# MKMaS-GUET/MTVAF

Measured on AMD Instinct MI355X. Metric: training sentences/sec (fwd+bwd), higher is better.
Workload: dtype fp32 (3xbf16 split products, fp32 accumulate)

## Files before the change

include/mtvaf_hip.h:

```cpp
#ifndef MTVAF_HIP_H
#define MTVAF_HIP_H

#include <stddef.h>
#include <stdint.h>

#ifdef __cplusplus
extern "C" {
#endif

typedef void* mtvaf_stream_t;

#define MTVAF_OK 0
#define MTVAF_ERR_SHAPE (-1)
#define MTVAF_ERR_ALIGN (-2)
#define MTVAF_ERR_ARG (-3)
#define MTVAF_ERR_WORKSPACE (-4)

#define MTVAF_KC 0
#define MTVAF_KM 1
#define MTVAF_EPI_NONE 0
#define MTVAF_EPI_GELU 1
#define MTVAF_EPI_TANH 2
#define MTVAF_EPI_DGELU 3
#define MTVAF_EPI_DTANH 4
// ... 265 lines not shown
typedef struct {
  float* dh;
  float* dh1;
  void *df, *dpre, *da, *dctx, *dqkv;
  float *part, *partq, *partkv;
  float* delta;
  float *dwqkv, *dbqkv, *dwo, *dbo, *dg1, *db1, *dw1, *dbi1, *dw2, *dbi2, *dg2, *db2;
  float *dpk, *dpv;
  void* ws_main; size_t ws_main_bytes;
  void* ws_side; size_t ws_side_bytes;
  const int* klist;
  const int* kcnt;
  int zero_tail;
  float *lnpart2, *lnpart1;
  void *df_p, *dpre_p, *da_p, *dqkv_p;
} mtvaf_layer_grads_t;

int mtvaf_encoder_layer_fwd(const mtvaf_layer_t* layer, mtvaf_stream_t stream);
int mtvaf_encoder_layer_bwd(const mtvaf_layer_t* layer, const mtvaf_layer_grads_t* grads, mtvaf_stream_t main,
                            mtvaf_stream_t side, int settle);
size_t mtvaf_layer_struct_bytes(int which );

int mtvaf_adamw(float* p, const float* g, float* m, float* v, long n, float lr, double beta1, double beta2, float eps,
                float weight_decay, float bc1, float bc2_sqrt, float grad_scale, void* p_bf16, int max_blocks,
                mtvaf_stream_t stream);
int mtvaf_adamw_planes(float* p, const float* g, float* m, float* v, long n, float lr, double beta1, double beta2, float eps,
                       float weight_decay, float bc1, float bc2_sqrt, float grad_scale, int nseg, const long* seg_begin,
                       const int* seg_rows, const int* seg_cols, void* const* seg_img, int max_blocks, mtvaf_stream_t stream);
int mtvaf_adamw_multi(int count, float* const* p, const float* const* g, float* const* m, float* const* v,
                      const long* n, float lr, double beta1, double beta2, float eps, float weight_decay, float bc1,
// ... 11 lines not shown
```

mtvaf_amd/csrc/executor.hip:

```cpp
#include "common.h"

#include <cstdlib>

#include <cstddef>

extern "C" {
int mtvaf_gemm_f32(int layout_a, int layout_b, const float* A, int lda, const float* B, int ldb, float* C, int ldc, int M,
                   int N, int K, const float* bias, int epi, float* aux, int ldaux, int accumulate, int allow_split,
                   void* workspace, size_t workspace_bytes, int cfg, int splits, hipStream_t stream);
int mtvaf_gemm_bf16x(int layout_a, int layout_b, const void* A, int lda, const void* B, int ldb, float* C32, int ldc32,
                     void* C16, int ldc16, int M, int N, int K, const float* bias, int epi, void* aux16, int ldaux,
                     int accumulate, float* colpart, int allow_split, void* workspace, size_t workspace_bytes, int tile,
                     int splits, int stages, hipStream_t stream);
int mtvaf_gemm_f32_dw_group(int n, const float* const* A, const int* lda, const float* const* B, const int* ldb, float* const* C,
                            const int* ldc, const int* M, const int* N, int K, const int* klist, const int* kcnt,
                            void* workspace, size_t workspace_bytes, int splits, hipStream_t stream);
int mtvaf_gemm_f32_dw_group_bias(int n, const float* const* A, const int* lda, const float* const* B, const int* ldb, float* const* C,
                                 const int* ldc, const int* M, const int* N, int K, const int* klist, const int* kcnt,
                                 float* const* dbias, void* workspace, size_t workspace_bytes, int splits, hipStream_t stream);
int mtvaf_streamk_attached(hipStream_t stream);
int mtvaf_gemm_bf16x_dw_group(int n, const void* const* A, const int* lda, const void* const* B, const int* ldb, float* const* C32,
                              const int* ldc32, const int* M, const int* N, int K, hipStream_t stream);
int mtvaf_gemm_bf16x_ktiles(int layout_a, int layout_b, const void* A, int lda, const void* B, int ldb, float* C32, int ldc32,
                            void* C16, int ldc16, int M, int N, int K, const float* bias, int epi, void* aux16, int ldaux,
// ... 190 lines not shown
struct mtvaf_layer_grads_t {
  float* dh;
  float* dh1;
  void *df, *dpre, *da, *dctx, *dqkv;
  float *part, *partq, *partkv;
  float* delta;
  float *dwqkv, *dbqkv, *dwo, *dbo, *dg1, *db1, *dw1, *dbi1, *dw2, *dbi2, *dg2, *db2;
  float *dpk, *dpv;
  void* ws_main; size_t ws_main_bytes;
  void* ws_side; size_t ws_side_bytes;
  const int* klist;
  const int* kcnt;
  int zero_tail;
  float *lnpart2, *lnpart1;
  void *df_p, *dpre_p, *da_p, *dqkv_p;
};

static int p16_ep(int lb, const void* Ap, const void* Wp, void* Cp, float* colpart, int M, int N, int K, const float* bias, int epi, float* aux,
                  int ldaux, hipStream_t st) {
  const long ap = (long)M * 64, akt = (long)3 * M * 64;
  const long bp = (long)(lb == 0 ? N : K) * 64, bkt = lb == 0 ? (long)3 * N * 64 : 2048, bc = lb == 0 ? 0 : (long)12 * K * 64;
  return mtvaf_gemm_f32p_ep(0, Ap, ap, 64, akt, 0, lb, Wp, bp, 64, bkt, bc, nullptr, 0, Cp, colpart, M, N, K, bias, epi, aux, ldaux, 0, st);
}

static bool planes_mode(const mtvaf_layer_t* L) {
  return !L->bf16 && L->cu && L->x_p && L->cx_p && L->h1_p && L->act_p && L->wqkv_h && L->wo_h && L->w1_h && L->w2_h && L->Mp % 128 == 0 &&
         L->H % 128 == 0 && L->I % 128 == 0 && L->ws;
}

static int dense_ln_fwd_p(const void* Ap, int K, const void* Wp, const float* bias, float* x_out, const float* res, const float* gamma,
                          const float* beta, float* out, float* mean, float* rstd, int M, int H, float eps, float p_drop, uint64_t seed,
// ... 120 lines not shown
                               nullptr, 0, nullptr, 0, 0, -1, 0, mainS));
    MTVAF_TRY(ln_bwd_forked(g->dh1, L->a, L->x, L->g1, L->mean1, L->rstd1, nullptr, g->dh, g->dg1, g->db1, g->dbo, M, H, L->p_hidden,
                            L->seed, L->offset + 1, g->lnpart1, g->ws_main, g->ws_main_bytes, g->da, mainS, side));
    if (!grp) MTVAF_TRY(mtvaf_gemm_bf16x_ktiles(X_KM, X_KM, g->da, H, L->cx, H, g->dwo, H, nullptr, 0, H, H, M, nullptr, X_EPI_NONE, nullptr, 0, 0,
                               nullptr, 1, g->ws_side, g->ws_side_bytes, 0, -1, 0, g->klist, g->kcnt, side));
    MTVAF_TRY(mtvaf_gemm_bf16x(X_KC, X_KM, g->da, H, L->wo_h, H, nullptr, 0, g->dctx, H, M, H, H, nullptr, X_EPI_NONE, nullptr, 0, 0,
                               nullptr, 0, nullptr, 0, 0, -1, 0, mainS));
    if (L->cu) {
      MTVAF_TRY(mtvaf_prefix_attn_bf16_varlen_bwd(g->dctx, L->qkv, L->pk, L->pv, L->cu, L->Mp - L->Mv, L->cx, L->lse, g->dqkv, g->dpk,
                                                  g->dpv, g->partq, g->partkv, B, S, P, NH, 64, L->p_attn, L->seed, L->offset, mainS));
    } else {
      MTVAF_TRY(mtvaf_prefix_attn_bf16_bwd_tail(g->dctx, L->qkv, L->pk, L->pv, L->addmask, L->cx, L->lse, g->dqkv, g->dpk, g->dpv, g->partq,
                                                g->partkv, B, S, P, NH, 64, L->p_attn, L->seed, L->offset,
                                                (g->klist != nullptr || g->zero_tail) ? 1 : 0, mainS));
    }
    MTVAF_TRY(fork_to(mainS, side));
    MTVAF_TRY(mtvaf_colsum_small(g->partq, B * ((S + 63) / 64), H, g->dbqkv, 0, side));
    MTVAF_TRY(mtvaf_colsum_small(g->partkv, B * ((P + S + 63) / 64), 2 * H, g->dbqkv + H, 0, side));
    if (!grp) MTVAF_TRY(mtvaf_gemm_bf16x_ktiles(X_KM, X_KM, g->dqkv, 3 * H, L->x_h, H, g->dwqkv, H, nullptr, 0, 3 * H, H, M, nullptr, X_EPI_NONE,
                               nullptr, 0, 0, nullptr, 1, g->ws_side, g->ws_side_bytes, 0, -1, 0, g->klist, g->kcnt, side));
    if (grp) {
      const void* const As[4] = {g->df, g->dpre, g->da, g->dqkv};
      const void* const Bs[4] = {L->act, L->h1_h, L->cx, L->x_h};
      float* const Cs[4] = {static_cast<float*>(g->dw2), static_cast<float*>(g->dw1), static_cast<float*>(g->dwo), static_cast<float*>(g->dwqkv)};
      const int lda[4] = {H, I, H, 3 * H}, ldb[4] = {I, H, H, H}, ldc[4] = {I, H, H, H};
      const int Ms[4] = {H, I, H, 3 * H}, Ns[4] = {I, H, H, H};
      MTVAF_TRY(mtvaf_gemm_bf16x_dw_group(4, As, lda, Bs, ldb, Cs, ldc, Ms, Ns, M, side));
    }
    MTVAF_TRY(mtvaf_gemm_bf16x(X_KC, X_KM, g->dqkv, 3 * H, L->wqkv_h, H, g->dh, H, nullptr, 0, M, H, 3 * H, nullptr, X_EPI_NONE,
                               nullptr, 0, 1, nullptr, 0, nullptr, 0, 0, -1, 0, mainS));
// ... 9 lines not shown
    const float* act = static_cast<const float*>(L->act);
    if (planes_mode(L)) {
      if (!g->df_p || !g->dpre_p || !g->da_p || !g->dqkv_p || !g->part || !g->lnpart2 || !g->lnpart1 || !g->ws_main) return MTVAF_ERR_ARG;
      MTVAF_TRY(mtvaf_dropout_res_ln_bwd_rows_planes(g->dh, nullptr, 0, L->f, L->h1, L->g2, L->mean2, L->rstd2, nullptr, g->dh1, 0, M, H,
                                                     L->p_hidden, L->seed, L->offset + 2, g->lnpart2, g->df_p, mainS));
      MTVAF_TRY(p16_ep(1, g->df_p, L->w2_h, g->dpre_p, g->part, M, I, H, nullptr, X_EPI_DGELU, pre, I, mainS));
      int ns1 = 1;
      MTVAF_TRY(p16(1, g->dpre_p, L->w1_h, g->dh1, H, M, H, I, nullptr, X_EPI_NONE, nullptr, 0, 1, g->ws_main, g->ws_main_bytes, &ns1, mainS));
      MTVAF_TRY(mtvaf_dropout_res_ln_bwd_rows_planes(g->dh1, static_cast<const float*>(g->ws_main), ns1 > 1 ? ns1 : 0, L->a, L->x, L->g1,
                                                     L->mean1, L->rstd1, nullptr, g->dh, 0, M, H, L->p_hidden, L->seed, L->offset + 1,
                                                     g->lnpart1, g->da_p, mainS));
      MTVAF_TRY(p16(1, g->da_p, L->wo_h, dctx, H, M, H, H, nullptr, X_EPI_NONE, nullptr, 0, 0, g->ws_main, g->ws_main_bytes, nullptr, mainS));
      MTVAF_TRY(mtvaf_prefix_attn_varlen_bwd_planes(dctx, qkv, static_cast<const float*>(L->pk), static_cast<const float*>(L->pv), L->cu,
                                                    L->Mp - L->Mv, cx, L->lse, g->delta, dqkv, g->dpk, g->dpv, B, S, P, NH, 64, L->p_attn,
                                                    L->seed, L->offset, g->dqkv_p, M, mainS));
      MTVAF_TRY(fork_to(mainS, side));
      {
        const void* const As[4] = {g->df_p, g->dpre_p, g->da_p, g->dqkv_p};
        const void* const Bs[4] = {L->act_p, L->h1_p, L->cx_p, L->x_p};
        float* const Cs[4] = {g->dw2, g->dw1, g->dwo, g->dwqkv};
        const int ldc[4] = {I, H, H, H}, Ms[4] = {H, I, H, 3 * H}, Ns[4] = {I, H, H, H};
        long strides[32];
        for (int i = 0; i < 8; ++i) {
          strides[4 * i] = (long)M * 64; strides[4 * i + 1] = 64; strides[4 * i + 2] = 2048; strides[4 * i + 3] = (long)12 * M * 64;
        }
        const float* js[8]; float* jd[8]; int jr[8], jc[8], jl[8], nj = 0;
        auto job = [&](const float* src, int rows, int cols, int ld, float* dst) {
          if (dst) { js[nj] = src; jr[nj] = rows; jc[nj] = cols; jl[nj] = ld; jd[nj] = dst; ++nj; }
        };
        job(dqkv, M, 3 * H, 3 * H, g->dbqkv);
// ... 37 lines not shown
                              L->offset + 1, g->lnpart1, g->ws_main, g->ws_main_bytes, nullptr, mainS, side));
    }
    if (!grp) MTVAF_TRY(mtvaf_gemm_f32_ktiles(X_KM, X_KM, da, H, cx, H, g->dwo, H, H, H, M, nullptr, X_EPI_NONE, nullptr, 0, 0, 1, g->ws_side,
                             g->ws_side_bytes, -1, -1, g->klist, g->kcnt, side));
    MTVAF_TRY(mtvaf_gemm_f32(X_KC, X_KM, da, H, L->wo, H, dctx, H, M, H, H, nullptr, X_EPI_NONE, nullptr, 0, 0, 1, g->ws_main,
                             g->ws_main_bytes, -1, -1, mainS));
    if (L->cu) {
      MTVAF_TRY(mtvaf_prefix_attn_varlen_bwd(dctx, qkv, static_cast<const float*>(L->pk), static_cast<const float*>(L->pv), L->cu,
                                             L->Mp - L->Mv, cx, L->lse, g->delta, dqkv, g->dpk, g->dpv, B, S, P, NH, 64, L->p_attn,
                                             L->seed, L->offset, mainS));
    } else {
      MTVAF_TRY(mtvaf_prefix_attn_bwd_tail(dctx, qkv, static_cast<const float*>(L->pk), static_cast<const float*>(L->pv), L->addmask, cx,
                                           L->lse, g->delta, dqkv, g->dpk, g->dpv, B, S, P, NH, 64, L->p_attn, L->seed, L->offset,
                                           (g->klist != nullptr || g->zero_tail) ? 1 : 0, mainS));
    }
    MTVAF_TRY(fork_to(mainS, side));
    if (!grp) MTVAF_TRY(mtvaf_colsum(dqkv, M, 3 * H, 3 * H, g->dbqkv, 0, g->ws_side, g->ws_side_bytes, side));
    if (!grp) MTVAF_TRY(mtvaf_gemm_f32_ktiles(X_KM, X_KM, dqkv, 3 * H, L->x, H, g->dwqkv, H, 3 * H, H, M, nullptr, X_EPI_NONE, nullptr, 0, 0, 1,
                             g->ws_side, g->ws_side_bytes, -1, -1, g->klist, g->kcnt, side));
    if (grp) {
      const float* const As[4] = {df, dpre, da, dqkv};
      const float* const Bs[4] = {act, static_cast<const float*>(L->h1), cx, static_cast<const float*>(L->x)};
      float* const Cs[4] = {g->dw2, g->dw1, g->dwo, g->dwqkv};
      const int lda[4] = {H, I, H, 3 * H}, ldb[4] = {I, H, H, H}, ldc[4] = {I, H, H, H};
      const int Ms[4] = {H, I, H, 3 * H}, Ns[4] = {I, H, H, H};
      float* const dbs[4] = {nullptr, g->dbi1, nullptr, g->dbqkv};
      MTVAF_TRY(mtvaf_gemm_f32_dw_group_bias(4, As, lda, Bs, ldb, Cs, ldc, Ms, Ns, M, g->klist, g->kcnt, dbs, g->ws_side, g->ws_side_bytes, -1,
                                             side));
    }
    MTVAF_TRY(mtvaf_gemm_f32(X_KC, X_KM, dqkv, 3 * H, L->wqkv, H, g->dh, H, M, H, 3 * H, nullptr, X_EPI_NONE, nullptr, 0, 1, 1,
// ... 10 lines not shown
```

mtvaf_amd/engine.py:

```python
from __future__ import annotations

import ctypes
import os
from typing import List, Optional

import torch

from . import hip



class _Rng:

    def __init__(self):
        self.offset = 0
        self.stream = 0

    def set_stream(self, stream: int):
        self.stream = int(stream)

    def seed(self) -> int:
        return (int(torch.initial_seed()) ^ (self.stream * 0x9E3779B97F4A7C15)) & 0xFFFFFFFFFFFFFFFF

    def next(self, n: int = 1) -> int:
# ... 174 lines not shown

N_LAYER_PARAMS = 16


DW_SIDE_STREAM = os.environ.get("MTVAF_DW_STREAM", "1") != "0"
DW_STREAM_MIN_ROWS = 1024
_side_streams = {}


def _side_stream(device) -> "torch.cuda.Stream":
    key = torch.device(device).index or 0
    st = _side_streams.get(key)
    if st is None:
        st = _side_streams[key] = torch.cuda.Stream(device=device)
    return st


NATIVE_EXEC = os.environ.get("MTVAF_NATIVE_EXEC", "1") != "0"
DIRECT_GRADS = os.environ.get("MTVAF_DIRECT_GRADS", "1") != "0"
UNPAD = os.environ.get("MTVAF_UNPAD", "1") != "0"


class padding_free:

    def __init__(self, on: bool):
        self.on = bool(on)

    def __enter__(self):
        global UNPAD
        self.was, UNPAD = UNPAD, self.on
# ... 315 lines not shown
    gviews = grad_sink.acquire(params) if grad_sink is not None else None
    if grad_sink is not None:
        grad_sink.token_rows = M
    direct = gviews is not None and DIRECT_GRADS and not _has_grad_hooks(params)
    if direct and _ddp_without_gradsync(grad_sink):
        direct = False
        if not _warned_ddp[0]:
            _warned_ddp[0] = True
            import warnings
            warnings.warn("mtvaf_amd: torch.distributed is initialised with several ranks but no mtvaf_amd.parallel.GradSync is attached "
                          "to this encoder; encoder gradients are returned through autograd (as with MTVAF_DIRECT_GRADS=0) so that a "
                          "DistributedDataParallel reducer sees them.  Use GradSync for the overlapped per-layer exchange.")
    pgrads: List[Optional[torch.Tensor]] = [None] * len(params)
    main = torch.cuda.current_stream()
    side = _side_stream(dev) if (DW_SIDE_STREAM and need_param_grads and M >= DW_STREAM_MIN_ROWS) else None
    main_h = hip._st()
    if side is not None:
        with torch.cuda.stream(side):
            side_h = hip._st()
            ws_side = hip.workspace(_exec_workspace_bytes(M, H, I, use_h), dev)
    else:
        side_h, ws_side = main_h, None
    ws_main = hip.workspace(_exec_workspace_bytes(M, H, I, use_h), dev)
    if ws_side is None:
        ws_side = ws_main
    if use_h and need_param_grads:
        _streamk_on(side, dev)
    (flay, _), (blay, btotal) = _fwd_layout(M, H, I, B, NH, S, use_h, planes), _bwd_layout(M, H, I, B, NH, S, Pn, use_h, planes)
    o_h2, o_h2h, o_h2p = dict(flay)["h2"], dict(flay)["h2_h"], dict(flay)["h2_p"]
    fn = hip.lib().mtvaf_encoder_layer_bwd
# ... 65 lines not shown
            gs = w._gst = hip.LayerGradsStruct()
        barena = torch.empty(btotal, dtype=torch.uint8, device=dev)
        keep.append(barena)
        bb = barena.data_ptr()
        for name, o in blay:
            setattr(gs, name, bb + o if o >= 0 else None)
        gs.dh = dh.data_ptr()
        gs.dwqkv, gs.dbqkv = dwqkv.data_ptr(), dbqkv.data_ptr()
        (gs.dwo, gs.dbo, gs.dg1, gs.db1, gs.dw1, gs.dbi1, gs.dw2, gs.dbi2, gs.dg2, gs.db2) = [t.data_ptr() for t in G[6:16]]
        gs.dpk = (dpk_ptr + li * dpk_layer) if Pn else None
        gs.dpv = (dpk_ptr + li * dpk_layer + dpk_step) if Pn else None
        gs.ws_main, gs.ws_main_bytes = ws_main.data_ptr(), ws_main.numel()
        gs.ws_side, gs.ws_side_bytes = ws_side.data_ptr(), ws_side.numel()
        gs.klist, gs.kcnt = (klist.data_ptr(), kcnt.data_ptr()) if klist is not None else (None, None)
        gs.zero_tail = int(zero_tail)
        hip._ck(fn(ctypes.byref(st), ctypes.byref(gs), main_h, side_h, settle), "mtvaf_encoder_layer_bwd")
        if gviews is None:
            G[0], G[2], G[4] = dwqkv[:H], dwqkv[H:2 * H], dwqkv[2 * H:]
            G[1], G[3], G[5] = dbqkv[:H], dbqkv[H:2 * H], dbqkv[2 * H:]
            keep.append((dwqkv, dbqkv))
        if direct:
            for p, gt in zip(params[base_i:base_i + N_LAYER_PARAMS], G):
                p.grad = gt
        else:
            pgrads[base_i:base_i + N_LAYER_PARAMS] = G
        if grad_sink is not None:
            if side is not None and grad_sink.on_layer_done is not None:
                if grad_sink.raw_stream_hook:
                    hip.STREAM_OVERRIDE = side_h
                    try:
                        grad_sink.layer_done(li)
# ... 113 lines not shown
        dev_like = flat[0]
        dpkv = torch.empty_like(pkv) if Pn else None
        need_param_grads = any(p.requires_grad for p in params)
        gviews = grad_sink.acquire(params) if grad_sink is not None else None
        if grad_sink is not None:
            grad_sink.token_rows = M
        pgrads: List[Optional[torch.Tensor]] = [None] * len(params)

        wh = ctx.wh
        use_h = wh is not None
        flat_t = flat[13 * L:]
        pkv16 = ctx.pkv16
        KC, KM = hip.KC, hip.KM
        main = torch.cuda.current_stream()
        side = _side_stream(dev_like.device) if (DW_SIDE_STREAM and need_param_grads and M >= DW_STREAM_MIN_ROWS) else None

        def on_side(reads, fn):
            if side is None:
                fn()
                return
            ev = torch.cuda.Event()
            ev.record(main)
            with torch.cuda.stream(side):
                side.wait_event(ev)
                fn()
            for t in reads:
                t.record_stream(side)

        zero_tail = bool(SKIP_PAD_DW and len(cfg) > 5 and cfg[5] and addmask.dtype == torch.float32 and addmask.is_contiguous())
        if CHECK_CONTRACT and zero_tail:
# ... 67 lines not shown
                hip.linear_bwd_input(dpre, w.w1, dh1, accumulate=True)
            dh0 = dh
            if use_h:
                da_h, dctx = _bf16(M, H, like=dev_like), _bf16(M, H, like=dev_like)
                hip.dropout_res_ln_bwd(dh1, a, x, w.g1, mean1, rstd1, None, dh0, False, G[8], G[9], False, p_hidden, seed,
                                       off + 1, dbias_x=G[7], dx16=da_h)
                if not grp:
                    on_side((da_h,), lambda: hip.gemm_bf16x(da_h, KM, cx, KM, H, H, M, out32=G[6], allow_split=True, ktiles=ktiles))
                hip.gemm_bf16x(da_h, KC, wo_h, KM, M, H, H, out16=dctx)
                dqkv = _bf16(M, 3 * H, like=dev_like)
                nqt, nkt = (S + 63) // 64, (Pn + S + 63) // 64
                partq, partkv = _empty(B * nqt, H, like=dev_like), _empty(B * nkt, 2 * H, like=dev_like)
                hip.prefix_attn_bf16_bwd(dctx, qkv, pkv16[li, 0] if Pn else None, pkv16[li, 1] if Pn else None, addmask, cx,
                                         lse, dqkv, dpkv[li, 0] if Pn else None, dpkv[li, 1] if Pn else None, partq, partkv,
                                         B, S, Pn, NH, p_attn, seed, off, zero_tail=zero_tail or ktiles is not None)

                def qkv_grads():
                    (hip.colsum_small if partq.shape[0] <= 256 else hip.colsum)(partq, dbqkv[:H])
                    (hip.colsum_small if partkv.shape[0] <= 256 else hip.colsum)(partkv, dbqkv[H:])
                    if grp:
                        hip.gemm_bf16x_dw_group([(df_h, act, G[12]), (dpre_h, h1_h, G[10]), (da_h, cx, G[6]), (dqkv, x_h, dwqkv)], M)
                    else:
                        hip.gemm_bf16x(dqkv, KM, x_h, KM, 3 * H, H, M, out32=dwqkv, allow_split=True, ktiles=ktiles)
                on_side((dqkv, partq, partkv, df_h, dpre_h, da_h), qkv_grads)
                hip.gemm_bf16x(dqkv, KC, wqkv_h, KM, M, H, 3 * H, out32=dh0, accumulate=True)
            else:
                dctx = dh1
                da = df if (side is None and not grp) else _empty(M, H, like=dev_like)
                hip.dropout_res_ln_bwd(dh1, a, x, w.g1, mean1, rstd1, da, dh0, False, G[8], G[9], False, p_hidden, seed,
                                       off + 1, dbias_x=G[7])
                if not grp:
                    on_side((da,), lambda: hip.linear_bwd_weight(da, cx, G[6], ktiles=ktiles))
                hip.linear_bwd_input(da, w.wo, dctx)
                dqkv, delta = _empty(M, 3 * H, like=dev_like), _empty(B, NH, S, like=dev_like)
                hip.prefix_attn_bwd(dctx, qkv, pkv[li, 0] if Pn else None, pkv[li, 1] if Pn else None, addmask, cx, lse,
                                    delta, dqkv, dpkv[li, 0] if Pn else None, dpkv[li, 1] if Pn else None, B, S, Pn, NH,
                                    p_attn, seed, off, zero_tail=zero_tail or ktiles is not None)

                def qkv_grads():
                    if grp:
                        hip.gemm_f32_dw_group([(df, act, G[12]), (dpre, h1, G[10]), (da, cx, G[6]), (dqkv, x, dwqkv)], M, ktiles=ktiles,
                                              dbias=[None, G[11], None, dbqkv])
                    else:
                        hip.colsum(dqkv, dbqkv)
                        hip.linear_bwd_weight(dqkv, x, dwqkv, ktiles=ktiles)
                on_side((dqkv, df, dpre, da) if grp else (dqkv,), qkv_grads)
                hip.linear_bwd_input(dqkv, w.wqkv, dh0, accumulate=True)
            dh = dh0
            if gviews is None:
                G[0], G[2], G[4] = dwqkv[:H], dwqkv[H:2 * H], dwqkv[2 * H:]
                G[1], G[3], G[5] = dbqkv[:H], dbqkv[H:2 * H], dbqkv[2 * H:]
            pgrads[base:base + N_LAYER_PARAMS] = G
# ... 90 lines not shown

    @staticmethod
    def backward(ctx, gout):
        em, start, end, trans, tags, mask_u8, ws, wsb = ctx.stash
        g = gout.contiguous().view(1).float()
        dem = torch.empty_like(em)
        ds, de, dt = torch.empty_like(start), torch.empty_like(end), torch.empty_like(trans)
        hip.crf_nll_bwd(g, em, tags, mask_u8, start, end, trans, dem, ds, de, dt, False, ws, wsb)
        return dem, ds, de, dt, None, None


class PromptFunction(torch.autograd.Function):

    @staticmethod
    def forward(ctx, enc, wp, bp, NL, *proj_params):
        NI, B, Lp, W4 = enc.shape
        W = W4 // 4
        n = NI * B
        encc = enc.contiguous()
        sm = _empty(n, Lp * W, like=encc)
        hip._ck(hip.lib().mtvaf_split_mean(hip._p(encc), hip._p(sm), n * Lp, W, hip._st()), "mtvaf_split_mean")
        logits = _empty(n, NL * 4, like=encc)
        hip.linear_fwd(sm, wp, bp, logits)
        gate = torch.empty_like(logits)
        hip._ck(hip.lib().mtvaf_gate_fwd(hip._p(logits), hip._p(gate), n * NL, hip._st()), "mtvaf_gate_fwd")
        pkv = _empty(NL, 2, B, NI * Lp * (W // 2), like=encc)
        hip._ck(hip.lib().mtvaf_prompt_mix_fwd(hip._p(encc), hip._p(gate), hip._p(pkv), NI, B, Lp, W, NL, hip._st()),
                "mtvaf_prompt_mix_fwd")
        ctx.stash = (encc, wp, sm, logits, gate, NL)
        ctx.proj_params = proj_params
        return pkv

    @staticmethod
    def backward(ctx, dpkv):
        encc, wp, sm, logits, gate, NL = ctx.stash
        NI, B, Lp, W4 = encc.shape
        W = W4 // 4
        n = NI * B
        dpkv = dpkv.contiguous()
        dpart = _empty(n * Lp, NL * 4, like=encc)
        dlog = _empty(n, NL * 4, like=encc)
        L_ = hip.lib()
        hip._ck(L_.mtvaf_prompt_mix_bwd_gate(hip._p(encc), hip._p(dpkv), hip._p(logits), hip._p(gate), hip._p(dpart),
                                             hip._p(dlog), NI, B, Lp, W, NL, hip._st()), "mtvaf_prompt_mix_bwd_gate")
        dwp = torch.empty_like(wp)
        hip.linear_bwd_weight(dlog, sm, dwp)
        dbp = _empty(NL * 4, like=encc)
        hip.colsum(dlog, dbp)
        dsm = torch.empty_like(sm)
        hip.linear_bwd_input(dlog, wp, dsm)
        denc = torch.empty_like(encc)
        hip._ck(L_.mtvaf_prompt_mix_bwd_enc(hip._p(gate), hip._p(dpkv), hip._p(dsm), hip._p(denc), NI, B, Lp, W, NL,
                                            hip._st()), "mtvaf_prompt_mix_bwd_enc")
        pg = []
        for i in range(NL):
            pg.append(dwp[4 * i:4 * i + 4])
            pg.append(dbp[4 * i:4 * i + 4])
        pp = ctx.proj_params
        if DIRECT_GRADS and all(p.requires_grad and p.grad is None for p in pp) and not _has_grad_hooks(pp):
            for p, g in zip(pp, pg):
                p.grad = g
            pg = [None] * len(pg)
        return (denc, None, None, None, *pg)


class MeanLFunction(torch.autograd.Function):

    @staticmethod
    def forward(ctx, enc):
        n, Lp, W4 = enc.shape
        e = enc.contiguous()
        out = _empty(n, W4, like=e)
        hip._ck(hip.lib().mtvaf_mean_l_fwd(hip._p(e), hip._p(out), n, Lp, W4, hip._st()), "mtvaf_mean_l_fwd")
        ctx.shape = (n, Lp, W4)
        return out

    @staticmethod
    def backward(ctx, dmean):
# ... 108 lines not shown
```

mtvaf_amd/hip.py:

```python
from __future__ import annotations

import ctypes
import os
from ctypes import c_double, c_float, c_int, c_int64, c_long, c_size_t, c_uint64, c_void_p
from typing import Optional

import torch

_HERE = os.path.dirname(os.path.abspath(__file__))
LIB_PATH = os.environ.get("MTVAF_LIB") or os.path.join(_HERE, "lib", "libmtvaf_hip.so")

_ERR = {-1: "bad shape", -2: "bad alignment", -3: "bad argument", -4: "workspace too small"}

P, I, L, F, U64, SZ = c_void_p, c_int, c_long, c_float, c_uint64, c_size_t

_SIGS = {
    "mtvaf_version": (c_int, []),
    "mtvaf_encoder_layer_fwd": (c_int, [P, P]),
    "mtvaf_encoder_layer_bwd": (c_int, [P, P, P, P, I]),
    "mtvaf_layer_struct_bytes": (SZ, [I]),
    "mtvaf_rng_set_epoch_ptr": (c_int, [P]),
    "mtvaf_rng_epoch_advance": (c_int, [P, P]),
    "mtvaf_device_cus": (c_int, []),
    "mtvaf_gemm_f32_workspace_bytes": (SZ, [I, I, I, I]),
# ... 99 lines not shown
                [(n, c_float) for n in ("eps", "p_hidden", "p_attn")] + [("seed", c_uint64), ("offset", c_uint64)] +
                [(n, c_void_p) for n in ("wqkv", "wo", "w1", "w2", "wqkv_h", "wo_h", "w1_h", "w2_h", "bqkv", "bo", "g1", "b1",
                                         "bi1", "bi2", "g2", "b2", "x", "x_h", "pk", "pv", "addmask", "qkv", "cx", "lse", "a",
                                         "h1", "h1_h", "mean1", "rstd1", "pre", "act", "f", "h2", "h2_h", "mean2", "rstd2",
                                         "ws")] + [("ws_bytes", c_size_t), ("cu", c_void_p), ("Mv", c_int), ("Mp", c_int)] +
                [(n, c_void_p) for n in ("x_p", "cx_p", "h1_p", "act_p", "h2_p")])


class LayerGradsStruct(ctypes.Structure):
    _fields_ = ([(n, c_void_p) for n in ("dh", "dh1", "df", "dpre", "da", "dctx", "dqkv", "part", "partq", "partkv", "delta",
                                         "dwqkv", "dbqkv", "dwo", "dbo", "dg1", "db1", "dw1", "dbi1", "dw2", "dbi2", "dg2",
                                         "db2", "dpk", "dpv", "ws_main")] + [("ws_main_bytes", c_size_t), ("ws_side", c_void_p),
                                                                            ("ws_side_bytes", c_size_t), ("klist", c_void_p),
                                                                            ("kcnt", c_void_p), ("zero_tail", c_int),
                                                                            ("lnpart2", c_void_p), ("lnpart1", c_void_p)] +
                [(n, c_void_p) for n in ("df_p", "dpre_p", "da_p", "dqkv_p")])


_lib = None


def lib():
    global _lib
    if _lib is None:
        if not os.path.exists(LIB_PATH):
            raise RuntimeError(
                f"mtvaf_amd: HIP extension {LIB_PATH} not found -- run `python -m mtvaf_amd.build` "
                "(there is no CPU fallback for the product path)")
        l = ctypes.CDLL(LIB_PATH)
        for name, (res, args) in _SIGS.items():
            fn = getattr(l, name)
# ... 665 lines not shown
```

mtvaf_amd/models/bert_model.py:

```python
from __future__ import annotations

from typing import List, Optional

import torch
from torch import nn
from transformers.modeling_outputs import TokenClassifierOutput

from .. import engine
from ..modules.crf import CRF
from .modeling_bert import BertModel, PrefixKV
from .modeling_roberta import RobertaModel


def _arg(args, name, default=False):
    return getattr(args, name, default)


def _on_second_stream(fn, inputs, join=False):
    ts = [t for t in inputs if isinstance(t, torch.Tensor)]
    if not (engine.DW_SIDE_STREAM and ts and ts[0].is_cuda and ts[0].shape[0] >= 8):
        return fn()
    main, side = torch.cuda.current_stream(), engine._side_stream(ts[0].device)
    side.wait_stream(main)
    _accumulate_on_producer_stream()
# ... 11 lines not shown
    return out


_warned_off = False


def _accumulate_on_producer_stream():
    global _warned_off
    if not _warned_off:
        _warned_off = True
        fn = getattr(torch.autograd.graph, "set_warn_on_accumulate_grad_stream_mismatch", None)
        if fn is not None:
            fn(False)


class ImageModel(nn.Module):

    def __init__(self, use_152=False, use_101=False, use_34=False, use_18=False, resnet_root=None):
        super().__init__()
        from .resnet import resnet18, resnet34, resnet50, resnet101, resnet152
        name, ctor = (("resnet152", resnet152) if use_152 else ("resnet101", resnet101) if use_101 else
                      ("resnet34", resnet34) if use_34 else ("resnet18", resnet18) if use_18 else ("resnet50", resnet50))
        self.resnet = ctor()
        if resnet_root is not None and resnet_root != "random":
            self.resnet.load_state_dict(torch.load(f"{resnet_root}/{name}.pth", map_location="cpu"))

    def forward(self, x, aux_imgs=None):
        prefix_guids = self.get_resnet_prompt(x)
        if aux_imgs is not None:
            aux_imgs = aux_imgs.permute([1, 0, 2, 3, 4])
# ... 130 lines not shown
            aux = [torch.cat(a, dim=1).view(bsz, L, -1) for a in (aux_pyr or [])]
            return feats.float(), [a.float() for a in aux]
        feats = images.reshape(bsz, L, -1).float()
        aux = []
        if aux_imgs is not None:
            aux = [aux_imgs[:, i].reshape(bsz, L, -1).float() for i in range(aux_imgs.shape[1])]
        return feats, aux

    def get_visual_prompt(self, images, aux_imgs, imagelabel):
        feats, aux = self._region_features(images, aux_imgs)
        bsz, L, Fd = feats.shape
        cfg = self.bert.config
        hidden = cfg.hidden_size
        NI = 1 + len(aux)
        x = torch.stack([feats] + aux).reshape(NI * bsz * L, Fd)
        e0, e2 = self.encoder_conv[0], self.encoder_conv[2]
        t = engine.LinearFunction.apply(x, e0.weight, e0.bias, True)
        enc = engine.LinearFunction.apply(t, e2.weight, e2.bias, False).view(NI, bsz, L, 8 * hidden)

        img_tag_loss = 0
        aux_img_tag_loss = []
        if _arg(self.args, "vao"):
            means = engine.MeanLFunction.apply(enc.view(NI * bsz, L, 8 * hidden)).view(NI, bsz, 8 * hidden)
            target = imagelabel.to(means.device)
            heads = [self.img_classifier] + list(self.aux_img_classifier)
            if NI - 1 > len(self.aux_img_classifier):
                raise ValueError("the VAO branch supports at most 3 aux images (bert_model.py:459)")
            for k in range(NI):
                m = engine.dropout(means[k], self.img_dropout.p, self.training)
                z = engine.LinearFunction.apply(m, heads[k].weight, heads[k].bias, False)
                l = engine.KLFunction.apply(z, target)
                if k == 0:
                    img_tag_loss = l
                else:
                    aux_img_tag_loss.append(l)

        if self._packed_proj is None or not self._packed_proj.valid(self.projectors):
            self._packed_proj = _PackedLinears(self.projectors)
        pp = self._packed_proj
        NL = len(self.projectors)
        proj_params = [p for m in self.projectors for p in (m.weight, m.bias)]
        pkv = engine.PromptFunction.apply(enc, pp.w, pp.b, NL, *proj_params)
        return PrefixKV(pkv, cfg.num_attention_heads, hidden // cfg.num_attention_heads), img_tag_loss, aux_img_tag_loss



def flatten(x):
    if x.dim() == 2:
        return x.reshape(x.shape[0] * x.shape[1])
    if x.dim() == 3:
# ... 97 lines not shown
    def classification(self, span_starts, span_ends, sequence_input, attention_mask):
        M = span_starts.shape[1]
        index = engine.hip.span_index(attention_mask.to(torch.uint8).contiguous(), span_starts.contiguous().long(),
                                      span_ends.contiguous().long())
        pooled = engine.SpanPoolFunction.apply(sequence_input, self.unary_affine.weight, self.unary_affine.bias, index, M)
        pooled = engine.LinearFunction.apply(pooled, self.dense.weight, self.dense.bias, True)
        pooled = engine.dropout(pooled, self.dropout.p, self.training)
        ac_logits = engine.LinearFunction.apply(pooled, self.classifier.weight, self.classifier.bias, False)
        return reconstruct(ac_logits, span_starts), ac_logits

    _region_features = TVNetSAModel2._region_features

    def get_visual_prompt(self, images, aux_imgs):
        feats, aux = self._region_features(images, aux_imgs)
        bsz, L, Fd = feats.shape
        cfg = self.bert.config
        hidden = cfg.hidden_size
        NI = 1 + len(aux)
        x = torch.stack([feats] + aux).reshape(NI * bsz * L, Fd)
        e0, e2 = self.encoder_conv[0], self.encoder_conv[2]
        t = engine.LinearFunction.apply(x, e0.weight, e0.bias, True)
        enc = engine.LinearFunction.apply(t, e2.weight, e2.bias, False).view(NI, bsz, L, 8 * hidden)
        if self._packed_proj is None or not self._packed_proj.valid(self.projectors):
            self._packed_proj = _PackedLinears(self.projectors)
        pp = self._packed_proj
        proj_params = [p for m in self.projectors for p in (m.weight, m.bias)]
        pkv = engine.PromptFunction.apply(enc, pp.w, pp.b, len(self.projectors), *proj_params)
        return PrefixKV(pkv, cfg.num_attention_heads, hidden // cfg.num_attention_heads)
```

Baseline: 3636.

## Overlap prompt-generator backward with encoder layer-0 backward via prefix-ready event

Records an event in the encoder layer-0 backward right after the prefix attention gradients (dpk/dpv) are produced, and files it keyed by the dpkv tensor. A new fused PromptGenFunction (encoder_conv linears plus the prompt mix) uses that event to start its backward on dedicated side streams. This lets the prompt-generator backward run while the rest of layer 0's backward (dW GEMMs, LN backward) is still executing, instead of waiting for it. The dW2 and db2 work is further forked onto a second stream. It adds cross-stream event bookkeeping and record_stream calls, and relies on version and pointer checks to stay correct.

After: 3633. No clear change (-0.1%).

```diff
diff --git a/include/mtvaf_hip.h b/include/mtvaf_hip.h
--- a/include/mtvaf_hip.h
+++ b/include/mtvaf_hip.h
@@ -303,6 +303,7 @@
   int zero_tail;
   float *lnpart2, *lnpart1;
   void *df_p, *dpre_p, *da_p, *dqkv_p;
+  void* prefix_ready;
 } mtvaf_layer_grads_t;
 
 int mtvaf_encoder_layer_fwd(const mtvaf_layer_t* layer, mtvaf_stream_t stream);
diff --git a/mtvaf_amd/csrc/executor.hip b/mtvaf_amd/csrc/executor.hip
--- a/mtvaf_amd/csrc/executor.hip
+++ b/mtvaf_amd/csrc/executor.hip
@@ -228,7 +228,14 @@
   int zero_tail;
   float *lnpart2, *lnpart1;
   void *df_p, *dpre_p, *da_p, *dqkv_p;
+  void* prefix_ready;
 };
+
+static int mark_prefix_ready(const mtvaf_layer_grads_t* g, hipStream_t mainS) {
+  if (!g->prefix_ready) return MTVAF_OK;
+  const hipError_t rc = hipEventRecord(static_cast<hipEvent_t>(g->prefix_ready), mainS);
+  return rc == hipSuccess ? MTVAF_OK : (int)rc;
+}
 
 static int p16_ep(int lb, const void* Ap, const void* Wp, void* Cp, float* colpart, int M, int N, int K, const float* bias, int epi, float* aux,
                   int ldaux, hipStream_t st) {
@@ -379,6 +386,7 @@
                                                 g->partkv, B, S, P, NH, 64, L->p_attn, L->seed, L->offset,
                                                 (g->klist != nullptr || g->zero_tail) ? 1 : 0, mainS));
     }
+    MTVAF_TRY(mark_prefix_ready(g, mainS));
     MTVAF_TRY(fork_to(mainS, side));
     MTVAF_TRY(mtvaf_colsum_small(g->partq, B * ((S + 63) / 64), H, g->dbqkv, 0, side));
     MTVAF_TRY(mtvaf_colsum_small(g->partkv, B * ((P + S + 63) / 64), 2 * H, g->dbqkv + H, 0, side));
@@ -418,6 +426,7 @@
       MTVAF_TRY(mtvaf_prefix_attn_varlen_bwd_planes(dctx, qkv, static_cast<const float*>(L->pk), static_cast<const float*>(L->pv), L->cu,
                                                     L->Mp - L->Mv, cx, L->lse, g->delta, dqkv, g->dpk, g->dpv, B, S, P, NH, 64, L->p_attn,
                                                     L->seed, L->offset, g->dqkv_p, M, mainS));
+      MTVAF_TRY(mark_prefix_ready(g, mainS));
       MTVAF_TRY(fork_to(mainS, side));
       {
         const void* const As[4] = {g->df_p, g->dpre_p, g->da_p, g->dqkv_p};
@@ -485,6 +494,7 @@
                                            L->lse, g->delta, dqkv, g->dpk, g->dpv, B, S, P, NH, 64, L->p_attn, L->seed, L->offset,
                                            (g->klist != nullptr || g->zero_tail) ? 1 : 0, mainS));
     }
+    MTVAF_TRY(mark_prefix_ready(g, mainS));
     MTVAF_TRY(fork_to(mainS, side));
     if (!grp) MTVAF_TRY(mtvaf_colsum(dqkv, M, 3 * H, 3 * H, g->dbqkv, 0, g->ws_side, g->ws_side_bytes, side));
     if (!grp) MTVAF_TRY(mtvaf_gemm_f32_ktiles(X_KM, X_KM, dqkv, 3 * H, L->x, H, g->dwqkv, H, 3 * H, H, M, nullptr, X_EPI_NONE, nullptr, 0, 0, 1,
diff --git a/mtvaf_amd/engine.py b/mtvaf_amd/engine.py
--- a/mtvaf_amd/engine.py
+++ b/mtvaf_amd/engine.py
@@ -212,6 +212,30 @@
     if st is None:
         st = _side_streams[key] = torch.cuda.Stream(device=device)
     return st
+
+
+_prefix_grad_ready = {}
+_prompt_streams = {}
+
+
+def _prompt_stream(device, i: int) -> "torch.cuda.Stream":
+    key = (torch.device(device).index or 0, i)
+    st = _prompt_streams.get(key)
+    if st is None:
+        st = _prompt_streams[key] = torch.cuda.Stream(device=device)
+    return st
+
+
+def _file_prefix_ready(dpkv, ev):
+    _prefix_grad_ready.clear()
+    _prefix_grad_ready[dpkv.data_ptr()] = (dpkv, dpkv._version, ev)
+
+
+def _take_prefix_ready(dpkv):
+    ent = _prefix_grad_ready.pop(dpkv.data_ptr(), None)
+    if ent is None or ent[0]._version != ent[1] or ent[0].untyped_storage().data_ptr() != dpkv.untyped_storage().data_ptr():
+        return None
+    return ent[2]
 
 
 NATIVE_EXEC = os.environ.get("MTVAF_NATIVE_EXEC", "1") != "0"
@@ -557,6 +581,10 @@
     pgrads: List[Optional[torch.Tensor]] = [None] * len(params)
     main = torch.cuda.current_stream()
     side = _side_stream(dev) if (DW_SIDE_STREAM and need_param_grads and M >= DW_STREAM_MIN_ROWS) else None
+    pready = None
+    if Pn and side is not None and ctx.needs_input_grad[1] and not torch.cuda.is_current_stream_capturing():
+        pready = torch.cuda.Event()
+        pready.record(main)
     main_h = hip._st()
     if side is not None:
         with torch.cuda.stream(side):
@@ -652,7 +680,10 @@
         gs.ws_side, gs.ws_side_bytes = ws_side.data_ptr(), ws_side.numel()
         gs.klist, gs.kcnt = (klist.data_ptr(), kcnt.data_ptr()) if klist is not None else (None, None)
         gs.zero_tail = int(zero_tail)
+        gs.prefix_ready = pready.cuda_event if (pready is not None and li == 0) else None
         hip._ck(fn(ctypes.byref(st), ctypes.byref(gs), main_h, side_h, settle), "mtvaf_encoder_layer_bwd")
+        if gs.prefix_ready:
+            _file_prefix_ready(dpkv, pready)
         if gviews is None:
             G[0], G[2], G[4] = dwqkv[:H], dwqkv[H:2 * H], dwqkv[2 * H:]
             G[1], G[3], G[5] = dbqkv[:H], dbqkv[H:2 * H], dbqkv[2 * H:]
@@ -796,6 +827,8 @@
         KC, KM = hip.KC, hip.KM
         main = torch.cuda.current_stream()
         side = _side_stream(dev_like.device) if (DW_SIDE_STREAM and need_param_grads and M >= DW_STREAM_MIN_ROWS) else None
+        pready = (torch.cuda.Event() if (Pn and side is not None and ctx.needs_input_grad[1] and not torch.cuda.is_current_stream_capturing())
+                  else None)
 
         def on_side(reads, fn):
             if side is None:
@@ -893,6 +926,9 @@
                 hip.prefix_attn_bf16_bwd(dctx, qkv, pkv16[li, 0] if Pn else None, pkv16[li, 1] if Pn else None, addmask, cx,
                                          lse, dqkv, dpkv[li, 0] if Pn else None, dpkv[li, 1] if Pn else None, partq, partkv,
                                          B, S, Pn, NH, p_attn, seed, off, zero_tail=zero_tail or ktiles is not None)
+                if pready is not None and li == 0:
+                    pready.record(main)
+                    _file_prefix_ready(dpkv, pready)
 
                 def qkv_grads():
                     (hip.colsum_small if partq.shape[0] <= 256 else hip.colsum)(partq, dbqkv[:H])
@@ -915,6 +951,9 @@
                 hip.prefix_attn_bwd(dctx, qkv, pkv[li, 0] if Pn else None, pkv[li, 1] if Pn else None, addmask, cx, lse,
                                     delta, dqkv, dpkv[li, 0] if Pn else None, dpkv[li, 1] if Pn else None, B, S, Pn, NH,
                                     p_attn, seed, off, zero_tail=zero_tail or ktiles is not None)
+                if pready is not None and li == 0:
+                    pready.record(main)
+                    _file_prefix_ready(dpkv, pready)
 
                 def qkv_grads():
                     if grp:
@@ -1035,54 +1074,137 @@
 
     @staticmethod
     def forward(ctx, enc, wp, bp, NL, *proj_params):
-        NI, B, Lp, W4 = enc.shape
-        W = W4 // 4
-        n = NI * B
-        encc = enc.contiguous()
-        sm = _empty(n, Lp * W, like=encc)
-        hip._ck(hip.lib().mtvaf_split_mean(hip._p(encc), hip._p(sm), n * Lp, W, hip._st()), "mtvaf_split_mean")
-        logits = _empty(n, NL * 4, like=encc)
-        hip.linear_fwd(sm, wp, bp, logits)
-        gate = torch.empty_like(logits)
-        hip._ck(hip.lib().mtvaf_gate_fwd(hip._p(logits), hip._p(gate), n * NL, hip._st()), "mtvaf_gate_fwd")
-        pkv = _empty(NL, 2, B, NI * Lp * (W // 2), like=encc)
-        hip._ck(hip.lib().mtvaf_prompt_mix_fwd(hip._p(encc), hip._p(gate), hip._p(pkv), NI, B, Lp, W, NL, hip._st()),
-                "mtvaf_prompt_mix_fwd")
-        ctx.stash = (encc, wp, sm, logits, gate, NL)
+        pkv, ctx.stash = _prompt_mix_fwd(enc, wp, bp, NL)
         ctx.proj_params = proj_params
         return pkv
 
     @staticmethod
     def backward(ctx, dpkv):
-        encc, wp, sm, logits, gate, NL = ctx.stash
-        NI, B, Lp, W4 = encc.shape
-        W = W4 // 4
-        n = NI * B
-        dpkv = dpkv.contiguous()
-        dpart = _empty(n * Lp, NL * 4, like=encc)
-        dlog = _empty(n, NL * 4, like=encc)
-        L_ = hip.lib()
-        hip._ck(L_.mtvaf_prompt_mix_bwd_gate(hip._p(encc), hip._p(dpkv), hip._p(logits), hip._p(gate), hip._p(dpart),
-                                             hip._p(dlog), NI, B, Lp, W, NL, hip._st()), "mtvaf_prompt_mix_bwd_gate")
-        dwp = torch.empty_like(wp)
-        hip.linear_bwd_weight(dlog, sm, dwp)
-        dbp = _empty(NL * 4, like=encc)
-        hip.colsum(dlog, dbp)
-        dsm = torch.empty_like(sm)
-        hip.linear_bwd_input(dlog, wp, dsm)
-        denc = torch.empty_like(encc)
-        hip._ck(L_.mtvaf_prompt_mix_bwd_enc(hip._p(gate), hip._p(dpkv), hip._p(dsm), hip._p(denc), NI, B, Lp, W, NL,
-                                            hip._st()), "mtvaf_prompt_mix_bwd_enc")
-        pg = []
-        for i in range(NL):
-            pg.append(dwp[4 * i:4 * i + 4])
-            pg.append(dbp[4 * i:4 * i + 4])
-        pp = ctx.proj_params
-        if DIRECT_GRADS and all(p.requires_grad and p.grad is None for p in pp) and not _has_grad_hooks(pp):
-            for p, g in zip(pp, pg):
-                p.grad = g
-            pg = [None] * len(pg)
-        return (denc, None, None, None, *pg)
+        denc, dwp, dbp = _prompt_mix_bwd(ctx.stash, dpkv)
+        return (denc, None, None, None, *_projector_grads(ctx.proj_params, dwp, dbp))
+
+
+def _prompt_mix_fwd(enc, wp, bp, NL):
+    NI, B, Lp, W4 = enc.shape
+    W = W4 // 4
+    n = NI * B
+    encc = enc.contiguous()
+    sm = _empty(n, Lp * W, like=encc)
+    hip._ck(hip.lib().mtvaf_split_mean(hip._p(encc), hip._p(sm), n * Lp, W, hip._st()), "mtvaf_split_mean")
+    logits = _empty(n, NL * 4, like=encc)
+    hip.linear_fwd(sm, wp, bp, logits)
+    gate = torch.empty_like(logits)
+    hip._ck(hip.lib().mtvaf_gate_fwd(hip._p(logits), hip._p(gate), n * NL, hip._st()), "mtvaf_gate_fwd")
+    pkv = _empty(NL, 2, B, NI * Lp * (W // 2), like=encc)
+    hip._ck(hip.lib().mtvaf_prompt_mix_fwd(hip._p(encc), hip._p(gate), hip._p(pkv), NI, B, Lp, W, NL, hip._st()),
+            "mtvaf_prompt_mix_fwd")
+    return pkv, (encc, wp, sm, logits, gate, NL)
+
+
+def _prompt_mix_bwd(stash, dpkv):
+    encc, wp, sm, logits, gate, NL = stash
+    NI, B, Lp, W4 = encc.shape
+    W = W4 // 4
+    n = NI * B
+    dpkv = dpkv.contiguous()
+    dpart = _empty(n * Lp, NL * 4, like=encc)
+    dlog = _empty(n, NL * 4, like=encc)
+    L_ = hip.lib()
+    hip._ck(L_.mtvaf_prompt_mix_bwd_gate(hip._p(encc), hip._p(dpkv), hip._p(logits), hip._p(gate), hip._p(dpart),
+                                         hip._p(dlog), NI, B, Lp, W, NL, hip._st()), "mtvaf_prompt_mix_bwd_gate")
+    dwp = torch.empty_like(wp)
+    hip.linear_bwd_weight(dlog, sm, dwp)
+    dbp = _empty(NL * 4, like=encc)
+    hip.colsum(dlog, dbp)
+    dsm = torch.empty_like(sm)
+    hip.linear_bwd_input(dlog, wp, dsm)
+    denc = torch.empty_like(encc)
+    hip._ck(L_.mtvaf_prompt_mix_bwd_enc(hip._p(gate), hip._p(dpkv), hip._p(dsm), hip._p(denc), NI, B, Lp, W, NL,
+                                        hip._st()), "mtvaf_prompt_mix_bwd_enc")
+    return denc, dwp, dbp
+
+
+def _projector_grads(pp, dwp, dbp):
+    pg = []
+    for i in range(len(pp) // 2):
+        pg.append(dwp[4 * i:4 * i + 4])
+        pg.append(dbp[4 * i:4 * i + 4])
+    if DIRECT_GRADS and all(p.requires_grad and p.grad is None for p in pp) and not _has_grad_hooks(pp):
+        for p, g in zip(pp, pg):
+            p.grad = g
+        pg = [None] * len(pg)
+    return pg
+
+
+class PromptGenFunction(torch.autograd.Function):
+
+    @staticmethod
+    def forward(ctx, x, w0, b0, w2, b2, shape, wp, bp, NL, *proj_params):
+        x = x.contiguous()
+        t = _empty(x.shape[0], w0.shape[0], like=x)
+        hip.linear_fwd(x, w0, b0, t, epi=hip.EPI_TANH)
+        enc = _empty(x.shape[0], w2.shape[0], like=x)
+        hip.linear_fwd(t, w2, b2, enc)
+        pkv, ctx.stash = _prompt_mix_fwd(enc.view(*shape, -1), wp, bp, NL)
+        ctx.gen = (x, w0, w2, t)
+        ctx.proj_params = proj_params
+        return pkv
+
+    @staticmethod
+    def backward(ctx, dpkv):
+        x, w0, w2, t = ctx.gen
+        need = ctx.needs_input_grad
+        ev = _take_prefix_ready(dpkv)
+        cur = torch.cuda.current_stream()
+        st = fork = None
+        if ev is not None:
+            st, fork = _prompt_stream(dpkv.device, 0), _prompt_stream(dpkv.device, 1)
+            st.wait_event(ev)
+            encc, _, sm, logits, gate, _ = ctx.stash
+            for u in (dpkv, x, t, encc, sm, logits, gate):
+                u.record_stream(st)
+        dx = dw0 = db0 = dw2 = db2 = None
+        with torch.cuda.stream(st):
+            denc, dwp, dbp = _prompt_mix_bwd(ctx.stash, dpkv)
+            dy = denc.view(-1, w2.shape[0])
+            if fork is not None:
+                forked = torch.cuda.Event()
+                forked.record(st)
+                fork.wait_event(forked)
+                denc.record_stream(fork)
+                t.record_stream(fork)
+            with torch.cuda.stream(fork):
+                if need[3]:
+                    dw2 = torch.empty_like(w2)
+                    hip.linear_bwd_weight(dy, t, dw2)
+                if need[4]:
+                    db2 = _empty(w2.shape[0], like=t)
+                    hip.colsum(dy, db2)
+            if need[0] or need[1] or need[2]:
+                dt = _empty(t.shape[0], t.shape[1], like=t)
+                hip.linear_bwd_input(dy, w2, dt)
+                dpre = torch.addcmul(dt, dt * t, t, value=-1.0)
+                if need[0]:
+                    dx = _empty(x.shape[0], x.shape[1], like=x)
+                    hip.linear_bwd_input(dpre, w0, dx)
+                if need[1]:
+                    dw0 = torch.empty_like(w0)
+                    hip.linear_bwd_weight(dpre, x, dw0)
+                if need[2]:
+                    db0 = _empty(w0.shape[0], like=x)
+                    hip.colsum(dpre, db0)
+            pg = _projector_grads(ctx.proj_params, dwp, dbp)
+        if st is not None:
+            joined = torch.cuda.Event()
+            joined.record(fork)
+            st.wait_event(joined)
+            done = torch.cuda.Event()
+            done.record(st)
+            cur.wait_event(done)
+            for g in (dx, dw0, db0, dw2, db2, dwp, dbp):
+                if g is not None:
+                    g.record_stream(cur)
+        return (dx, dw0, db0, dw2, db2, None, None, None, None, *pg)
 
 
 class MeanLFunction(torch.autograd.Function):
diff --git a/mtvaf_amd/hip.py b/mtvaf_amd/hip.py
--- a/mtvaf_amd/hip.py
+++ b/mtvaf_amd/hip.py
@@ -137,7 +137,7 @@
                                                                             ("ws_side_bytes", c_size_t), ("klist", c_void_p),
                                                                             ("kcnt", c_void_p), ("zero_tail", c_int),
                                                                             ("lnpart2", c_void_p), ("lnpart1", c_void_p)] +
-                [(n, c_void_p) for n in ("df_p", "dpre_p", "da_p", "dqkv_p")])
+                [(n, c_void_p) for n in ("df_p", "dpre_p", "da_p", "dqkv_p", "prefix_ready")])
 
 
 _lib = None
diff --git a/mtvaf_amd/models/bert_model.py b/mtvaf_amd/models/bert_model.py
--- a/mtvaf_amd/models/bert_model.py
+++ b/mtvaf_amd/models/bert_model.py
@@ -49,6 +49,18 @@
             fn(False)
 
 
+def _prompt_generator(model, x, shape) -> PrefixKV:
+    if model._packed_proj is None or not model._packed_proj.valid(model.projectors):
+        model._packed_proj = _PackedLinears(model.projectors)
+    pp = model._packed_proj
+    e0, e2 = model.encoder_conv[0], model.encoder_conv[2]
+    proj_params = [p for m in model.projectors for p in (m.weight, m.bias)]
+    pkv = engine.PromptGenFunction.apply(x, e0.weight, e0.bias, e2.weight, e2.bias, shape, pp.w, pp.b, len(model.projectors),
+                                         *proj_params)
+    cfg = model.bert.config
+    return PrefixKV(pkv, cfg.num_attention_heads, cfg.hidden_size // cfg.num_attention_heads)
+
+
 class ImageModel(nn.Module):
 
     def __init__(self, use_152=False, use_101=False, use_34=False, use_18=False, resnet_root=None):
@@ -209,26 +221,26 @@
         hidden = cfg.hidden_size
         NI = 1 + len(aux)
         x = torch.stack([feats] + aux).reshape(NI * bsz * L, Fd)
+        if not _arg(self.args, "vao"):
+            return _prompt_generator(self, x, (NI, bsz, L)), 0, []
         e0, e2 = self.encoder_conv[0], self.encoder_conv[2]
         t = engine.LinearFunction.apply(x, e0.weight, e0.bias, True)
         enc = engine.LinearFunction.apply(t, e2.weight, e2.bias, False).view(NI, bsz, L, 8 * hidden)
 
-        img_tag_loss = 0
         aux_img_tag_loss = []
-        if _arg(self.args, "vao"):
-            means = engine.MeanLFunction.apply(enc.view(NI * bsz, L, 8 * hidden)).view(NI, bsz, 8 * hidden)
-            target = imagelabel.to(means.device)
-            heads = [self.img_classifier] + list(self.aux_img_classifier)
-            if NI - 1 > len(self.aux_img_classifier):
-                raise ValueError("the VAO branch supports at most 3 aux images (bert_model.py:459)")
-            for k in range(NI):
-                m = engine.dropout(means[k], self.img_dropout.p, self.training)
-                z = engine.LinearFunction.apply(m, heads[k].weight, heads[k].bias, False)
-                l = engine.KLFunction.apply(z, target)
-                if k == 0:
-                    img_tag_loss = l
-                else:
-                    aux_img_tag_loss.append(l)
+        means = engine.MeanLFunction.apply(enc.view(NI * bsz, L, 8 * hidden)).view(NI, bsz, 8 * hidden)
+        target = imagelabel.to(means.device)
+        heads = [self.img_classifier] + list(self.aux_img_classifier)
+        if NI - 1 > len(self.aux_img_classifier):
+            raise ValueError("the VAO branch supports at most 3 aux images (bert_model.py:459)")
+        for k in range(NI):
+            m = engine.dropout(means[k], self.img_dropout.p, self.training)
+            z = engine.LinearFunction.apply(m, heads[k].weight, heads[k].bias, False)
+            l = engine.KLFunction.apply(z, target)
+            if k == 0:
+                img_tag_loss = l
+            else:
+                aux_img_tag_loss.append(l)
 
         if self._packed_proj is None or not self._packed_proj.valid(self.projectors):
             self._packed_proj = _PackedLinears(self.projectors)
@@ -356,16 +368,6 @@
     def get_visual_prompt(self, images, aux_imgs):
         feats, aux = self._region_features(images, aux_imgs)
         bsz, L, Fd = feats.shape
-        cfg = self.bert.config
-        hidden = cfg.hidden_size
         NI = 1 + len(aux)
         x = torch.stack([feats] + aux).reshape(NI * bsz * L, Fd)
-        e0, e2 = self.encoder_conv[0], self.encoder_conv[2]
-        t = engine.LinearFunction.apply(x, e0.weight, e0.bias, True)
-        enc = engine.LinearFunction.apply(t, e2.weight, e2.bias, False).view(NI, bsz, L, 8 * hidden)
-        if self._packed_proj is None or not self._packed_proj.valid(self.projectors):
-            self._packed_proj = _PackedLinears(self.projectors)
-        pp = self._packed_proj
-        proj_params = [p for m in self.projectors for p in (m.weight, m.bias)]
-        pkv = engine.PromptFunction.apply(enc, pp.w, pp.b, len(self.projectors), *proj_params)
-        return PrefixKV(pkv, cfg.num_attention_heads, hidden // cfg.num_attention_heads)
+        return _prompt_generator(self, x, (NI, bsz, L))
```
